# SciSharp/Gym.NET

Measured on AMD Instinct MI355X. Metric: env-steps/sec, higher is better.
Workload: dtype f32

## Files before the change

### gym.net_amd/build.py

```python
import os
import shutil
import subprocess

HERE = os.path.dirname(os.path.abspath(__file__))
CSRC = os.path.join(HERE, "csrc")
OUT = os.path.join(HERE, "lib", "libgymnet_amd.so")
SOURCES = ["env_cartpole.hip", "env_cartpole64.hip", "env_acrobot.hip", "env_pendulum.hip", "env_mountaincar.hip",
           "env_mountaincar_continuous.hip", "kernels.hip", "capi.hip", "launch_policy.hip", "resident.hip", "step_graph.hip",
           "group.hip", "render.hip", "pixel_stack.hip", "episode_memory.hip", "actor.hip", "actor_box.hip", "actor_box_policy.hip", "actor_box_logd.hip",
           "actor_softmax.hip", "actor_logp.hip", "actor_value.hip", "action_repeat.hip", "advantage.hip", "rollout_fused.hip"]
DEPS = SOURCES + ["kernels.hpp", "step_kernels.hpp", "lanes.hpp", "envs.hpp", "cartpole64.hpp", "philox.hpp", "handle.hpp", "launch_policy.hpp", "rollout_plan.hpp", "cartpole_raster.hpp", "actor_net.hpp", "actor_compose_logp.hpp", "actor_box_compose.hpp", "exp_neg.hpp", "log_pos.hpp", "advantage.hpp",
                  os.path.join("..", "..", "include", "gymnet_amd.h")]
FLAGS = ["--offload-arch=gfx950", "-O3", "-std=c++17", "-ffp-contract=off", "-fno-slp-vectorize", "-mllvm", "-amdgpu-kernarg-preload-count=14",
         "-fPIC", "-shared"]
LIBS = ["-ldl"]


def hipcc():
    exe = shutil.which("hipcc") or "/opt/rocm/bin/hipcc"
    if not os.path.exists(exe):
        raise RuntimeError("hipcc not found: cannot build the HIP extension")
    return exe


def up_to_date():
    if not os.path.exists(OUT):
        return False
    t = os.path.getmtime(OUT)
    return all(os.path.getmtime(os.path.join(CSRC, d)) <= t for d in DEPS)


def build(force=False, verbose=False):
    if not force and up_to_date():
        return OUT
    os.makedirs(os.path.dirname(OUT), exist_ok=True)
    import concurrent.futures
    import tempfile
    compile_flags = [f for f in FLAGS if f != "-shared"]
    with tempfile.TemporaryDirectory(prefix="gymnet_build_") as tmp:
        def compile_one(src):
            obj = os.path.join(tmp, os.path.splitext(src)[0] + ".o")
            cmd = [hipcc()] + compile_flags + ["-c", os.path.join(CSRC, src), "-o", obj]
            r = subprocess.run(cmd, capture_output=True, text=True)
            if r.returncode != 0:
                raise RuntimeError("hipcc failed:\n" + " ".join(cmd) + "\n" + r.stdout + r.stderr)
            return obj
        with concurrent.futures.ThreadPoolExecutor(max_workers=len(SOURCES)) as pool:
            objs = list(pool.map(compile_one, SOURCES))
        cmd = [hipcc(), "--offload-arch=gfx950", "-fPIC", "-shared"] + objs + LIBS + ["-o", OUT + ".tmp"]
        r = subprocess.run(cmd, capture_output=True, text=True)
        if r.returncode != 0:
            raise RuntimeError("hipcc (link) failed:\n" + " ".join(cmd) + "\n" + r.stdout + r.stderr)
    os.replace(OUT + ".tmp", OUT)
    if verbose:
        print("built", OUT)
    return OUT


if __name__ == "__main__":
    build(force=True, verbose=True)
```

### gym.net_amd/csrc/envs.hpp

```cpp
#pragma once
#include <hip/hip_runtime.h>
#include <stdint.h>

#include "philox.hpp"

namespace gymnet {


typedef float f2 __attribute__((ext_vector_type(2)));
namespace vm {
__device__ __forceinline__ float splat(float, float v) { return v; }
__device__ __forceinline__ f2 splat(f2, float v) { return f2{v, v}; }
__device__ __forceinline__ float fma(float a, float b, float c) { return fmaf(a, b, c); }
__device__ __forceinline__ f2 fma(f2 a, f2 b, f2 c) { return __builtin_elementwise_fma(a, b, c); }
template <class T> __device__ __forceinline__ T fmak(float k, T b, T c) { return fma(splat(b, k), b, c); }
template <class T> __device__ __forceinline__ T fmac(T a, T b, float k) { return fma(a, b, splat(a, k)); }
}

__device__ __forceinline__ void sincos_quadrant(float s, float c, float n, float &s_out, float &c_out) {
    const uint32_t q = (uint32_t)(int)n;
    const uint32_t q30 = q << 30, q31 = q << 31;
    const bool odd = (int32_t)q31 < 0;
    const float ss = odd ? c : s, cc = odd ? s : c;
    s_out = __uint_as_float(__builtin_amdgcn_bitop3_b32(__float_as_uint(ss), q30, 0x80000000u, 0x78));
    c_out = __uint_as_float(__builtin_amdgcn_bitop3_b32(__float_as_uint(cc), q30 ^ q31, 0x80000000u, 0x78));
}

template <class T>
__device__ __forceinline__ void sincos_bounded(T x, T &s_out, T &c_out) {
    T n;
    const T xs = x * vm::splat(x, 0.636619772367581343f);
    if constexpr (sizeof(T) == sizeof(float)) n = rintf(xs);
    else n = T{rintf(xs.x), rintf(xs.y)};
    T r = vm::fmak(-1.5703125f, n, x);
    r = vm::fmak(-4.837512969970703125e-4f, n, r);
    r = vm::fmak(-7.54978995489188216e-8f, n, r);
    const T z = r * r;
    T ps = vm::fmac(vm::splat(z, -1.9515295891e-4f), z, 8.3321608736e-3f);
    ps = vm::fmac(ps, z, -1.6666654611e-1f);
    const T s = vm::fma(r * z, ps, r);
    T pc = vm::fmac(vm::splat(z, 2.443315711809948e-5f), z, -1.388731625493765e-3f);
    pc = vm::fmac(pc, z, 4.166664568298827e-2f);
    const T c = vm::fma(z * z, pc, vm::fmac(vm::splat(z, -0.5f), z, 1.0f));
    if constexpr (sizeof(T) == sizeof(float)) {
        sincos_quadrant(s, c, n, s_out, c_out);
    } else {
        float s0, c0, s1, c1;
        sincos_quadrant(s.x, c.x, n.x, s0, c0);
        sincos_quadrant(s.y, c.y, n.y, s1, c1);
        s_out = T{s0, s1};
        c_out = T{c0, c1};
    }
}

template <class T>
__device__ __forceinline__ void sincos_small(T x, T &s_out, T &c_out) {
    T n;
    const T xs = x * vm::splat(x, 0.636619772367581343f);
    if constexpr (sizeof(T) == sizeof(float)) n = rintf(xs);
    else n = T{rintf(xs.x), rintf(xs.y)};
    T r = vm::fmak(-0x1.921fap+0f, n, x);
    r = vm::fmak(-0x1.54442ep-20f, n, r);
    const T z = r * r;
    T ps = vm::fmac(vm::splat(z, -1.9515295891e-4f), z, 8.3321608736e-3f);
    ps = vm::fmac(ps, z, -1.6666654611e-1f);
    const T s = vm::fma(r * z, ps, r);
    T pc = vm::fmac(vm::splat(z, 2.443315711809948e-5f), z, -1.388731625493765e-3f);
    pc = vm::fmac(pc, z, 4.166664568298827e-2f);
    pc = vm::fmac(pc, z, -0.5f);
    const T c = vm::fmac(pc, z, 1.0f);
    if constexpr (sizeof(T) == sizeof(float)) {
        sincos_quadrant(s, c, n, s_out, c_out);
    } else {
        float s0, c0, s1, c1;
        sincos_quadrant(s.x, c.x, n.x, s0, c0);
        sincos_quadrant(s.y, c.y, n.y, s1, c1);
        s_out = T{s0, s1};
        c_out = T{c0, c1};
    }
}

constexpr float kSmallAngle = 0.785f;
__device__ __forceinline__ void sincos_tiny(float x, float &s_out, float &c_out) {
    const float z = x * x;
    float ps = fmaf(-1.9515295891e-4f, z, 8.3321608736e-3f);
    ps = fmaf(ps, z, -1.6666654611e-1f);
// ... 38 lines not shown
    static constexpr const char *NAME = "CartPole";
    static constexpr int32_t ACTION_N = 2;

    static constexpr float gravity = 9.8f;
    static constexpr float masspole = 0.1f;
    static constexpr float total_mass = 0.1f + 1.0f;
    static constexpr float length = 0.5f;
    static constexpr float polemass_length = 0.1f * 0.5f;
    static constexpr float force_mag = 10.0f;
    static constexpr float tau = 0.02f;
    static constexpr float theta_threshold = 0.20943951606750488f;
    static constexpr float x_threshold = 2.4f;

    __device__ __forceinline__ static float div_tm(float x) { return DivByTotalMass<>::apply(x); }

    static constexpr bool HAS_SMALL_ANGLE_PATH = true;
    static constexpr int ANGLE_ROW = 2;
    static constexpr float SMALL_ANGLE_BOUND = kSmallAngle;

    template <bool SMALL_ANGLE = false, bool AUTORESET = false>
    __device__ __forceinline__ static void step(float (&s)[S], Action a, float &reward, bool &done) {
        const float x = s[0], x_dot = s[1], theta = s[2], theta_dot = s[3];
        const float s_in[S] = {x, x_dot, theta, theta_dot};
        const float force = (a == 1) ? force_mag : -force_mag;
        float sintheta, costheta;
        if constexpr (SMALL_ANGLE) sincos_tiny(theta, sintheta, costheta);
        else sincos_f32(theta, sintheta, costheta);
        const float temp = div_tm(force + polemass_length * theta_dot * theta_dot * sintheta);
        const float thetaacc = (gravity * sintheta - costheta * temp)
                               / (length * (4.0f / 3.0f - div_tm(masspole * costheta * costheta)));
        const float xacc = temp - div_tm(polemass_length * thetaacc * costheta);
        const float nx = x + tau * x_dot;
        const float nx_dot = x_dot + tau * xacc;
        const float ntheta = theta + tau * theta_dot;
        const float ntheta_dot = theta_dot + tau * thetaacc;
        s[0] = nx; s[1] = nx_dot; s[2] = ntheta; s[3] = ntheta_dot;
        bool term[DONE_TERMS];
        done_terms_of_inputs(s_in, term);
        done = term[0] || term[1];
        reward = 1.0f;
    }

    struct Pre {
        float x_dot, theta_dot;
        float nx, ntheta;
        float costheta;
        float centrifugal;
        float gsin;
        float divisor;
    };
    template <bool SMALL_ANGLE = false>
    __device__ __forceinline__ static void step_pre(const float (&s)[S], Pre &p) {
        const float x = s[0], x_dot = s[1], theta = s[2], theta_dot = s[3];
        float sintheta, costheta;
        if constexpr (SMALL_ANGLE) sincos_tiny(theta, sintheta, costheta);
        else sincos_f32(theta, sintheta, costheta);
        p.centrifugal = polemass_length * theta_dot * theta_dot * sintheta;
        p.gsin = gravity * sintheta;
        p.divisor = length * (4.0f / 3.0f - div_tm(masspole * costheta * costheta));
        p.costheta = costheta;
        p.nx = x + tau * x_dot;
        p.ntheta = theta + tau * theta_dot;
        p.x_dot = x_dot;
        p.theta_dot = theta_dot;
    }
    __device__ __forceinline__ static void step_post(const Pre &p, Action a, float (&s)[S], float &reward) { step_post(p, a == 1, s, reward); }
    __device__ __forceinline__ static void step_post(const Pre &p, bool right, float (&s)[S], float &reward) {
        const float force = right ? force_mag : -force_mag;
        const float temp = div_tm(force + p.centrifugal);
        const float thetaacc = (p.gsin - p.costheta * temp) / p.divisor;
        const float xacc = temp - div_tm(polemass_length * thetaacc * p.costheta);
        s[0] = p.nx; s[1] = p.x_dot + tau * xacc; s[2] = p.ntheta; s[3] = p.theta_dot + tau * thetaacc;
        reward = 1.0f;
    }

    static constexpr int DONE_TERMS = 2;
    __device__ __forceinline__ static void done_terms_of_inputs(const float (&s)[S], bool (&term)[DONE_TERMS]) {
        const double vx = __builtin_fma((double)tau, (double)s[1], (double)s[0]);
        const double vtheta = __builtin_fma((double)tau, (double)s[3], (double)s[2]);
        term[0] = __builtin_fabs(vx) > (double)x_threshold;
        term[1] = __builtin_fabs(vtheta) > (double)theta_threshold;
    }

    __device__ __forceinline__ static void reset(float (&s)[S], const PhiloxWords &r) {
#pragma unroll
        for (int k = 0; k < 4; ++k) s[k] = -0.05f + 0.1f * u01_24(r.w[k]);
    }

    __device__ __forceinline__ static void observe(const float (&s)[S], float (&o)[O]) {
#pragma unroll
        for (int k = 0; k < 4; ++k) o[k] = s[k];
    }
    __device__ __forceinline__ static void observe_fresh(const float (&s)[S], float (&o)[O]) { observe(s, o); }
    __device__ __forceinline__ static void step_observe(float (&s)[S], Action a, float &reward, bool &done, float (&o)[O]) {
        step(s, a, reward, done);
        observe(s, o);
    }
};

struct Pendulum {
    static constexpr int S = 2;
    static constexpr int O = 3;
    static constexpr bool OBS_ALIASES_STATE = false;
    static constexpr int OBS_ROW_OF_STATE[S] = {-1, 2};
    static constexpr bool HAS_SBD = false;
    static constexpr bool BOX_ACTION = true;
    static constexpr bool PACKED2 = false;
    static constexpr bool PIPE_LANES = false, PIPE_PAIRS = false;
    static constexpr bool HAS_SMALL_ANGLE_PATH = false;
    using Action = float;
    using Real = float;
    static constexpr bool RESET_TAKES_KEY = false;
    static constexpr const char *NAME = "Pendulum";
    static constexpr float ACTION_LOW = -2.0f, ACTION_HIGH = 2.0f;
    static constexpr float PI = 3.14159265358979323846f;

    __device__ __forceinline__ static float fmod_2pi(float a) {
        constexpr float m = 2.0f * PI, inv_m = 1.0f / m;
        const float ax = fabsf(a);
        if (__builtin_expect(!(ax < 4194304.0f * m), 0)) return fmodf(a, m);
        float q = truncf(ax * inv_m);
        float r = fmaf(-q, m, ax);
        q = r < 0.0f ? q - 1.0f : (r >= m ? q + 1.0f : q);
        r = fmaf(-q, m, ax);
        return copysignf(r, a);
    }

    __device__ __forceinline__ static float floored_mod_2pi(float a) {
        float r = fmod_2pi(a);
        if (r < 0.0f) r += 2.0f * PI;
        return r;
    }

    __device__ __forceinline__ static void step(float (&s)[S], Action a, float &reward, bool &done) {
        const float max_speed = 8.0f, max_torque = 2.0f, dt = 0.05f;
        const float th = s[0], thdot = s[1];
        const float u = a < -max_torque ? -max_torque : (a > max_torque ? max_torque : a);
        const float nrm = floored_mod_2pi(th + PI) - PI;
        const float costs = nrm * nrm + 0.1f * (thdot * thdot) + 0.001f * (u * u);
        float newthdot = thdot + (15.0f * sin_f32(th) + 3.0f * u) * dt;
        newthdot = newthdot < -max_speed ? -max_speed : (newthdot > max_speed ? max_speed : newthdot);
        const float newth = th + newthdot * dt;
        s[0] = newth; s[1] = newthdot;
        reward = -costs;
        done = false;
    }

    __device__ __forceinline__ static void reset(float (&s)[S], const PhiloxWords &r) {
        s[0] = -PI + (2.0f * PI) * u01_24(r.w[0]);
        s[1] = -1.0f + 2.0f * u01_24(r.w[1]);
    }

    __device__ __forceinline__ static void observe(const float (&s)[S], float (&o)[O]) {
        float sn, cs;
        sincos_f32(s[0], sn, cs);
        o[0] = cs; o[1] = sn; o[2] = s[1];
    }
    __device__ __forceinline__ static void observe_fresh(const float (&s)[S], float (&o)[O]) { observe(s, o); }
    __device__ __forceinline__ static void step_observe(float (&s)[S], Action a, float &reward, bool &done, float (&o)[O]) {
        step(s, a, reward, done);
        observe(s, o);
    }
};

struct MountainCar {
    static constexpr int S = 2;
// ... 231 lines not shown
```

### gym.net_amd/csrc/step_kernels.hpp

```cpp
#pragma once
#include "kernels.hpp"

#include <cstdio>
#include <type_traits>

#include "lanes.hpp"
#include "philox.hpp"

namespace gymnet {

__device__ __forceinline__ float abs_real(float x) { return fabsf(x); }
__device__ __forceinline__ double abs_real(double x) { return __builtin_fabs(x); }

template <class Env, bool UNIFORM_KEY = false>
__device__ __forceinline__ void draw_reset(typename Env::Real (&s)[Env::S], uint64_t key, uint64_t lane, uint64_t tick) {
    if constexpr (Env::RESET_TAKES_KEY) Env::reset(s, key, lane, tick);
    else Env::reset(s, lane_words<UNIFORM_KEY>(key, lane, tick));
}

template <class Env>
__device__ __forceinline__ constexpr bool state_row_own(int k) {
    if constexpr (Env::OBS_ALIASES_STATE) return true; else return Env::OBS_ROW_OF_STATE[k] < 0;
}
template <class Env>
// ... 2 lines not shown
    if constexpr (Env::OBS_ALIASES_STATE) return state + k * state_stride;
    else return Env::OBS_ROW_OF_STATE[k] < 0 ? state + k * state_stride : obs_in + Env::OBS_ROW_OF_STATE[k] * obs_stride;
}

__device__ __forceinline__ uint32_t wave_shard() {
    return (uint32_t)((((int64_t)blockIdx.x * blockDim.x + threadIdx.x) >> 6) & (kShards - 1));
}

template <int VEC, class Args>
__device__ __forceinline__ void count_after_done(const Args &a, const bool (&after)[VEC]) {
    uint32_t total = 0;
#pragma unroll
    for (int j = 0; j < VEC; ++j) total += (uint32_t)__popcll(__ballot(after[j]));
    if (total && lane_id() == (uint32_t)(__ffsll((unsigned long long)__ballot(1)) - 1))
        atomicAdd(&a.after_done[wave_shard() * kAfterStride], (unsigned long long)total);
}

template <class Env, bool AUTORESET, bool SMALL_ANGLE = false>
__device__ __forceinline__ void advance_sublane(typename Env::Real (&sj)[Env::S], typename Env::Action act, int32_t &sbd, float &rw,
                                                bool &dn, bool &after, bool in_range, typename Env::Real (&oj)[Env::O]) {
    if constexpr (Env::HAS_SMALL_ANGLE_PATH) Env::template step<SMALL_ANGLE, AUTORESET>(sj, act, rw, dn);
    else if constexpr (Env::OBS_ALIASES_STATE) Env::step(sj, act, rw, dn);
    else Env::step_observe(sj, act, rw, dn, oj);
    if constexpr (!AUTORESET && Env::HAS_SBD) {
        if (dn) {
            if (sbd == -1) { sbd = 0; }
            else { after = in_range; sbd += 1; rw = 0.0f; }
        }
    }
}

template <class Env, int VEC>
__device__ __forceinline__ bool wave_angles_small(const typename Env::Real (&s)[Env::S][VEC]) {
    if constexpr (!Env::HAS_SMALL_ANGLE_PATH) return false;
    else {
        bool small = true;
#pragma unroll
        for (int j = 0; j < VEC; ++j) small = small && (abs_real(s[Env::ANGLE_ROW][j]) <= Env::SMALL_ANGLE_BOUND);
        return __ballot(!small) == 0;
    }
}

template <class Env, int VEC, bool AUTORESET, bool GUARD, bool PACK = true>
__device__ __forceinline__ void advance_all(typename Env::Real (&s)[Env::S][VEC], typename Env::Action (&act)[VEC], int32_t (&sbd)[VEC],
                                            float (&rw)[VEC], bool (&dn)[VEC], bool (&after)[VEC], typename Env::Real (&o)[Env::O][VEC],
                                            int64_t i0, int64_t n) {
    constexpr int S = Env::S, O = Env::O;
    using Real = typename Env::Real;
#ifndef GYMNET_PROBE_NO_PACK
    constexpr bool kPack = true;
#else
    constexpr bool kPack = false;
#endif
    if constexpr (Env::PACKED2 && VEC == 2 && kPack && PACK) {
        Env::step_observe_x2(s, act, rw, dn, o);
    } else {
        auto all_sublanes = [&](auto small_tag) {
#pragma unroll
            for (int j = 0; j < VEC; ++j) {
                Real sj[S], oj[O];
#pragma unroll
                for (int k = 0; k < S; ++k) sj[k] = s[k][j];
                advance_sublane<Env, AUTORESET, decltype(small_tag)::value>(sj, act[j], sbd[j], rw[j], dn[j], after[j], !GUARD || i0 + j < n, oj);
#pragma unroll
                for (int k = 0; k < S; ++k) s[k][j] = sj[k];
                if constexpr (!Env::OBS_ALIASES_STATE) {
#pragma unroll
                    for (int k = 0; k < O; ++k) o[k][j] = oj[k];
                }
            }
        };
        if constexpr (Env::HAS_SMALL_ANGLE_PATH) {
            if (wave_angles_small<Env, VEC>(s)) all_sublanes(std::true_type{});
            else all_sublanes(std::false_type{});
        } else {
            all_sublanes(std::false_type{});
        }
    }
}

template <class Env, class = void> struct has_done_of_inputs : std::false_type {};
template <class Env> struct has_done_of_inputs<Env, std::void_t<decltype(&Env::done_terms_of_inputs)>> : std::true_type {};

template <class Env, class = void> struct has_split_step : std::false_type {};
template <class Env> struct has_split_step<Env, std::void_t<typename Env::Pre>> : std::true_type {};

template <class Env, int VEC>
__device__ __forceinline__ void pre_all_late_done(const typename Env::Real (&s)[Env::S][VEC], typename Env::Pre (&pre)[VEC], bool (&dn)[VEC],
                                                  uint64_t (&dmask)[VEC]) {
    constexpr int S = Env::S;
    using Real = typename Env::Real;
    static_assert(Env::HAS_SMALL_ANGLE_PATH && Env::OBS_ALIASES_STATE && has_done_of_inputs<Env>::value && has_split_step<Env>::value, "see above");
    auto all_sublanes = [&](auto small_tag) {
#pragma unroll
        for (int j = 0; j < VEC; ++j) {
            Real sj[S];
#pragma unroll
            for (int k = 0; k < S; ++k) sj[k] = s[k][j];
            Env::template step_pre<decltype(small_tag)::value>(sj, pre[j]);
        }
    };
    if (wave_angles_small<Env, VEC>(s)) all_sublanes(std::true_type{});
    else all_sublanes(std::false_type{});
#pragma unroll
    for (int j = 0; j < VEC; ++j) {
        Real wj[S];
#pragma unroll
        for (int k = 0; k < S; ++k) wj[k] = s[k][j];
        bool term[Env::DONE_TERMS];
        Env::done_terms_of_inputs(wj, term);
        bool any = false;
        uint64_t m = 0;
#pragma unroll
        for (int q = 0; q < Env::DONE_TERMS; ++q) { any = any || term[q]; m |= __builtin_amdgcn_ballot_w64(term[q]); }
        dn[j] = any;
        dmask[j] = m;
    }
}

template <class Env, int VEC>
__device__ __forceinline__ void post_all(const typename Env::Pre (&pre)[VEC], const typename Env::Action (&act)[VEC], const uint64_t (&dmask)[VEC],
                                         typename Env::Real (&s)[Env::S][VEC], float (&rw)[VEC]) {
    constexpr int S = Env::S;
    static_assert(std::is_same<typename Env::Action, int32_t>::value, "a discrete action");
    int32_t one = 1;
#pragma unroll
    for (int jj = 0; jj < VEC; ++jj) asm volatile("" : "+s"(one) : "v"(pre[jj].divisor), "s"(dmask[jj]));
#pragma unroll
    for (int j = 0; j < VEC; ++j) {
        typename Env::Real sj[S];
        Env::step_post(pre[j], act[j] == one, sj, rw[j]);
#pragma unroll
        for (int k = 0; k < S; ++k) s[k][j] = sj[k];
    }
}

template <class Env, int VEC, bool LANE_SEEDS>
__device__ __forceinline__ void reset_pending(uint32_t pending, typename Env::Real (&s)[Env::S][VEC], typename Env::Real (&o)[Env::O][VEC],
                                              const StepArgsT<typename Env::Real> &a, int64_t i0, int64_t n, uint64_t tick) {
    constexpr int S = Env::S, O = Env::O;
    using Real = typename Env::Real;
    while (pending) {
        const int j = __ffs(pending) - 1;
        pending &= pending - 1;
        Real sj[S];
        bool drawn = false;
        if constexpr (LANE_SEEDS) {
            if (a.lane_seed) {
                draw_reset<Env, false>(sj, i0 + j < n ? a.lane_seed[i0 + j] : a.seed, a.lane_offset + (uint64_t)(i0 + j), tick);
                drawn = true;
            }
        }
        if (!drawn) draw_reset<Env, true>(sj, a.seed, a.lane_offset + (uint64_t)(i0 + j), tick);
        Real oj[O];
        if constexpr (!Env::OBS_ALIASES_STATE) Env::observe_fresh(sj, oj);
#pragma unroll
        for (int jj = 0; jj < VEC; ++jj) {
            if (jj == j) {
#pragma unroll
                for (int k = 0; k < S; ++k) s[k][jj] = sj[k];
                if constexpr (!Env::OBS_ALIASES_STATE) {
#pragma unroll
                    for (int k = 0; k < O; ++k) o[k][jj] = oj[k];
                }
            }
        }
    }
}

template <class Env>
constexpr bool has_split_reset() { return Env::RESET_TAKES_KEY && Env::OBS_ALIASES_STATE; }

__device__ __forceinline__ PhiloxWords neighbour_words(const PhiloxWords &w) {
    PhiloxWords o;
#pragma unroll
    for (int k = 0; k < 4; ++k) o.w[k] = (uint32_t)__builtin_amdgcn_mov_dpp((int)w.w[k], 0xB1, 0xF, 0xF, true);
    return o;
}

#ifdef GYMNET_PROBE_RESET_MASKED
constexpr bool kResetFullExec = false;
#else
constexpr bool kResetFullExec = true;
#endif

template <class Env>
struct ResetScratch {
    uint32_t slot[64];
    typename Env::Real draw[64][Env::S];
};

__device__ __forceinline__ void wave_lds_fence() {
    __builtin_amdgcn_fence(__ATOMIC_RELEASE, "wavefront");
    __builtin_amdgcn_wave_barrier();
    __builtin_amdgcn_fence(__ATOMIC_ACQUIRE, "wavefront");
}

template <class Env, int VEC, bool LANE_SEEDS>
__device__ __forceinline__ void reset_pending_wave(uint32_t pending, typename Env::Real (&s)[Env::S][VEC], const StepArgsT<typename Env::Real> &a,
                                                   int64_t i0, int64_t n, uint64_t tick, ResetScratch<Env> *sc) {
// ... 28 lines not shown
        wave_lds_fence();
        if constexpr (SPLIT) {
            const uint32_t r = lane >> 1, call = lane & 1u;
            const bool draws = r < A && r < total - base;
            PhiloxWords w{};
            if (kResetFullExec || draws) {
                const uint32_t sl = sc->slot[draws ? r : 0u];
                const int64_t gl = wave_i0 + (int64_t)sl;
                uint64_t key = a.seed;
                if constexpr (LANE_SEEDS) {
                    if (a.lane_seed && gl < n) key = a.lane_seed[gl];
                }
                w = lane_words(Env::reset_call_key(key, call), a.lane_offset + (uint64_t)gl, tick);
            }
            const PhiloxWords other = neighbour_words(w);
            if ((kResetFullExec || draws) && call == 0) {
                Real sj[S];
                Env::reset_from_words(sj, w, other);
#pragma unroll
                for (int k = 0; k < S; ++k) sc->draw[r][k] = sj[k];
            }
        } else if (kResetFullExec || lane < total - base) {
            const uint32_t sl = sc->slot[lane < total - base ? lane : 0u];
            const int64_t gl = wave_i0 + (int64_t)sl;
            Real sj[S];
            bool drawn = false;
            if constexpr (LANE_SEEDS) {
                if (a.lane_seed) {
                    draw_reset<Env, false>(sj, gl < n ? a.lane_seed[gl] : a.seed, a.lane_offset + (uint64_t)gl, tick);
                    drawn = true;
                }
            }
            if (!drawn) draw_reset<Env, true>(sj, a.seed, a.lane_offset + (uint64_t)gl, tick);
#pragma unroll
            for (int k = 0; k < S; ++k) sc->draw[lane][k] = sj[k];
        }
        wave_lds_fence();
        Real got[VEC][S];
#pragma unroll
        for (int j = 0; j < VEC; ++j) {
            const uint32_t r = rank[j] - base;
#pragma unroll
            for (int k = 0; k < S; ++k) got[j][k] = sc->draw[r < A ? r : 0u][k];
        }
#pragma unroll
        for (int j = 0; j < VEC; ++j) {
            const bool mine = ((pending >> j) & 1u) && rank[j] - base < A;
#pragma unroll
            for (int k = 0; k < S; ++k) s[k][j] = mine ? got[j][k] : s[k][j];
        }
        wave_lds_fence();
    }
}

template <int VEC>
struct FinishedRanks {
    uint32_t rank[VEC];
    uint32_t total;
    bool single;
};

template <class Env, int VEC, bool LANE_SEEDS>
__device__ __forceinline__ void reset_finished_draw(const bool (&fin)[VEC], const uint64_t (&fmask)[VEC], const StepArgsT<typename Env::Real> &a,
                                                    int64_t wave_i0, int64_t n, uint64_t tick, ResetScratch<Env> *sc, FinishedRanks<VEC> &fr) {
    constexpr int S = Env::S;
    using Real = typename Env::Real;
    static_assert(Env::OBS_ALIASES_STATE && !has_split_reset<Env>(), "one-call resets that hand back the state only");
    const uint32_t lane = lane_id();
    uint32_t total = 0;
#pragma unroll
    for (int j = 0; j < VEC; ++j) {
        const uint64_t m = fmask[j];
        fr.rank[j] = total + __builtin_amdgcn_mbcnt_hi((uint32_t)(m >> 32), __builtin_amdgcn_mbcnt_lo((uint32_t)m, 0u));
        total += (uint32_t)__popcll(m);
    }
    fr.total = total;
    fr.single = !__builtin_expect(total == 0 || total > 64u || __ballot(1) != ~0ull, 0);
    if (!fr.single) return;
#pragma unroll
    for (int j = 0; j < VEC; ++j)
        if (fin[j]) sc->slot[fr.rank[j]] = lane * VEC + (uint32_t)j;
    wave_lds_fence();
    {
        const uint32_t sl = sc->slot[lane < total ? lane : 0u];
        const int64_t gl = wave_i0 + (int64_t)sl;
        Real sj[S];
        bool drawn = false;
        if constexpr (LANE_SEEDS) {
            if (a.lane_seed) {
                draw_reset<Env, false>(sj, gl < n ? a.lane_seed[gl] : a.seed, a.lane_offset + (uint64_t)gl, tick);
                drawn = true;
            }
        }
        if (!drawn) draw_reset<Env, true>(sj, a.seed, a.lane_offset + (uint64_t)gl, tick);
#pragma unroll
        for (int k = 0; k < S; ++k) sc->draw[lane][k] = sj[k];
    }
    wave_lds_fence();
}

template <class Env, int VEC>
__device__ __forceinline__ void reset_finished_take(const bool (&fin)[VEC], const FinishedRanks<VEC> &fr, typename Env::Real (&s)[Env::S][VEC],
                                                    ResetScratch<Env> *sc) {
    constexpr int S = Env::S;
    using Real = typename Env::Real;
    Real got[VEC][S];
#pragma unroll
    for (int j = 0; j < VEC; ++j) {
#pragma unroll
        for (int k = 0; k < S; ++k) got[j][k] = sc->draw[fr.rank[j] & 63u][k];
    }
#pragma unroll
    for (int j = 0; j < VEC; ++j) {
#pragma unroll
        for (int k = 0; k < S; ++k) s[k][j] = fin[j] ? got[j][k] : s[k][j];
    }
    wave_lds_fence();
}

template <class Env, int VEC, bool LANE_SEEDS>
__device__ __forceinline__ void reset_finished_rest(const bool (&fin)[VEC], const FinishedRanks<VEC> &fr, typename Env::Real (&s)[Env::S][VEC],
                                                    const StepArgsT<typename Env::Real> &a, int64_t i0, int64_t n, uint64_t tick, ResetScratch<Env> *sc) {
    if (fr.total == 0) return;
    uint32_t pending = 0;
#pragma unroll
    for (int j = 0; j < VEC; ++j) pending |= fin[j] ? (1u << j) : 0u;
    reset_pending_wave<Env, VEC, LANE_SEEDS>(pending, s, a, i0, n, tick, sc);
}

template <int VEC>
__device__ __forceinline__ uint32_t rank_finished(const bool (&finished)[VEC], uint32_t (&off)[VEC]) {
    uint32_t total = 0;
#pragma unroll
    for (int j = 0; j < VEC; ++j) {
        const uint64_t m = __ballot(finished[j]);
        off[j] = total + __builtin_amdgcn_mbcnt_hi((uint32_t)(m >> 32), __builtin_amdgcn_mbcnt_lo((uint32_t)m, 0u));
        total += (uint32_t)__popcll(m);
    }
    return total;
}

template <class Env, int VEC>
__device__ __forceinline__ void append_done_records(const StepArgsT<typename Env::Real> &a, const bool (&finished)[VEC], int64_t i0,
                                                    const typename Env::Real (&s)[Env::S][VEC], const typename Env::Real (&o)[Env::O][VEC],
                                                    const float (&fin_ret)[VEC], const int32_t (&fin_len)[VEC], bool stats) {
    constexpr int S = Env::S, O = Env::O;
    const uint32_t lane = lane_id();
    uint32_t off[VEC];
    const uint32_t total = rank_finished<VEC>(finished, off);
    if (total) {
        const int leader = __ffsll((unsigned long long)__ballot(1)) - 1;
        const uint32_t shard = wave_shard();
        uint32_t base = 0;
        if ((int)lane == leader)
            base = atomicAdd(&a.done_count2[a.cparity * (kShards * kCountStride) + shard * kCountStride], total);
        base = __shfl(base, leader);
        const int64_t seg0 = (int64_t)shard * a.done_cap;
#pragma unroll
        for (int j = 0; j < VEC; ++j) {
            if (!finished[j]) continue;
            const int64_t pos = seg0 + base + off[j];
            a.done_list[pos] = (int32_t)(i0 + j);
            if (stats) { a.rec_ret[pos] = fin_ret[j]; a.rec_len[pos] = fin_len[j]; }
            if (a.rec_obs) {
#pragma unroll
                for (int k = 0; k < O; ++k)
                    a.rec_obs[((int64_t)shard * O + k) * a.done_cap + base + off[j]] = Env::OBS_ALIASES_STATE ? s[k < S ? k : 0][j] : o[k][j];
// ... 102 lines not shown
                ep_len[j] += 1;
                if (a.max_episode_steps > 0 && ep_len[j] >= a.max_episode_steps) db |= 2;
            }
        }
        const bool fin = db != 0;
        finished[j] = fin && (!GUARD || i0 + j < n);
        done[j] = db;
        reward[j] = rw;

        if constexpr (EXTRAS) {
            if (fin && a.final_obs && (!GUARD || i0 + j < n)) {
#pragma unroll
                for (int k = 0; k < O; ++k) a.final_obs[k * n + i0 + j] = Env::OBS_ALIASES_STATE ? s[k < S ? k : 0][j] : o[k][j];
            }
            if (stats && fin && (!GUARD || i0 + j < n)) {
                fin_ret[j] = ep_ret[j];
                fin_len[j] = ep_len[j];
                if (a.fin_ret) { a.fin_ret[i0 + j] = ep_ret[j]; a.fin_len[i0 + j] = ep_len[j]; }
                if constexpr (AUTORESET) { ep_ret[j] = 0.0f; ep_len[j] = 0; }
            }
        }

        if constexpr (AUTORESET) pending |= fin ? (1u << j) : 0u;
    }

    if constexpr (!AUTORESET && Env::HAS_SBD) count_after_done<VEC>(a, after);

    store_f32<VEC, NT_O, GUARD>(a.reward, i0, n, reward);
    store_u8<VEC, NT_O, GUARD>(a.done, i0, n, done);

    if constexpr (EXTRAS) {
        if (a.done_list) append_done_records<Env, VEC>(a, finished, i0, s, o, fin_ret, fin_len, stats);
    }

    if constexpr (AUTORESET && RESETF == 1) reset_pending_wave<Env, VEC, EXTRAS>(pending, s, a, i0, n, tick, sc);
    else if constexpr (AUTORESET) reset_pending<Env, VEC, EXTRAS>(pending, s, o, a, i0, n, tick);

#pragma unroll
    for (int k = 0; k < S; ++k)
        if (state_row_own<Env>(k)) store_row<Real, VEC, NT_SS, GUARD>(a.state_out + k * a.state_stride, i0, n, s[k]);
    if constexpr (!Env::OBS_ALIASES_STATE) {
#pragma unroll
        for (int k = 0; k < O; ++k) store_row<Real, VEC, NT_SS, GUARD>(a.obs + k * a.obs_stride, i0, n, o[k]);
    }
    if constexpr (!AUTORESET && Env::HAS_SBD) store_i32<VEC, NT_SS, GUARD>(a.sbd, i0, n, sbd);

    if constexpr (EXTRAS) {
        if (stats) { store_f32<VEC, NT_SS, GUARD>(a.ep_ret, i0, n, ep_ret); store_i32<VEC, NT_SS, GUARD>(a.ep_len, i0, n, ep_len); }
    }
}

template <class Env, int VEC, bool AUTORESET, bool EXTRAS, int NT, bool GUARD, int RESETF = 0>
__device__ __forceinline__ void step_body(const StepArgsT<typename Env::Real> &a, const int64_t i0, const uint64_t tick, ResetScratch<Env> *sc = nullptr) {
    LaneInputs<Env, VEC> in;
    load_inputs<Env, VEC, AUTORESET, NT, GUARD>(a, i0, in);
    advance_and_store<Env, VEC, AUTORESET, EXTRAS, NT, GUARD, RESETF>(a, i0, tick, in, sc);
}

template <class Env, bool AUTORESET, bool EXTRAS>
constexpr bool has_full_workgroup_body() {
    return AUTORESET && !EXTRAS && Env::HAS_SMALL_ANGLE_PATH && Env::OBS_ALIASES_STATE && !has_split_reset<Env>() && has_done_of_inputs<Env>::value &&
           has_split_step<Env>::value;
}

template <class T>
__device__ __forceinline__ T *wg_row(T *row, const WgLanes &wg) { return wave_uniform(row + wg.first); }

#ifdef GYMNET_PROBE_RESET_BEHIND_ACTION
constexpr bool kResetDrawAhead = false;
#else
constexpr bool kResetDrawAhead = true;
#endif

template <class Env, int VEC, int NT, int RESETF>
__device__ __forceinline__ void step_body_wg(const StepArgsT<typename Env::Real> &a, const WgLanes wg, const uint64_t tick, ResetScratch<Env> *sc) {
    constexpr int S = Env::S;
    using Real = typename Env::Real;
    constexpr bool NT_SL = (NT & 1) != 0, NT_SS = (NT & 2) != 0, NT_A = (NT & 4) != 0, NT_O = (NT & 8) != 0;
    static_assert(!Env::BOX_ACTION && Env::OBS_ALIASES_STATE, "a discrete-action env whose observation is its state");
    const int64_t i0 = wg.first + (int64_t)wg.local;

    Real s[S][VEC];
    typename Env::Action act[VEC];
#pragma unroll
    for (int k = 0; k < S; ++k) load_row_wg<Real, VEC, NT_SL>(wg_row(static_cast<const Real *>(a.state) + k * a.state_stride, wg), wg.local, s[k]);
    load_row_wg<int32_t, VEC, NT_A>(wg_row(static_cast<const int32_t *>(a.action), wg), wg.local, act);

    typename Env::Pre pre[VEC];
    bool finished[VEC];
    uint64_t fmask[VEC];
    pre_all_late_done<Env, VEC>(s, pre, finished, fmask);

    float reward[VEC];
    auto store_reward_done = [&] {
        const uint32_t local = reissued(wg.local);
        store_row_wg<float, VEC, NT_O>(wg_row(a.reward, wg), local, reward);
        uint32_t w = 0;
#pragma unroll
        for (int j = 0; j < VEC; ++j) w |= finished[j] ? (1u << (8 * j)) : 0u;
        store_done_word_wg<VEC, NT_O>(wg_row(a.done, wg), local, w);
    };

    if constexpr (RESETF == 1 && kResetDrawAhead) {
        FinishedRanks<VEC> fr;
        reset_finished_draw<Env, VEC, false>(finished, fmask, a, wg.first + (int64_t)__builtin_amdgcn_readfirstlane(wg.local), a.n, tick, sc, fr);
        if (fr.single) {
            post_all<Env, VEC>(pre, act, fmask, s, reward);
            reset_finished_take<Env, VEC>(finished, fr, s, sc);
        } else {
            post_all<Env, VEC>(pre, act, fmask, s, reward);
            reset_finished_rest<Env, VEC, false>(finished, fr, s, a, wg.first + (int64_t)reissued(wg.local), a.n, tick, sc);
        }
        store_reward_done();
    } else {
        post_all<Env, VEC>(pre, act, fmask, s, reward);
        store_reward_done();
        if constexpr (RESETF == 1) {
            FinishedRanks<VEC> fr;
            reset_finished_draw<Env, VEC, false>(finished, fmask, a, wg.first + (int64_t)__builtin_amdgcn_readfirstlane(wg.local), a.n, tick, sc, fr);
            if (fr.single) reset_finished_take<Env, VEC>(finished, fr, s, sc);
            else reset_finished_rest<Env, VEC, false>(finished, fr, s, a, i0, a.n, tick, sc);
        } else {
            uint32_t pending = 0;
#pragma unroll
            for (int j = 0; j < VEC; ++j) pending |= finished[j] ? (1u << j) : 0u;
            Real o_unused[Env::O][VEC];
            reset_pending<Env, VEC, false>(pending, s, o_unused, a, i0, a.n, tick);
        }
    }

    const uint32_t local = reissued(wg.local);
#pragma unroll
    for (int k = 0; k < S; ++k) store_row_wg<Real, VEC, NT_SS>(wg_row(a.state_out + k * a.state_stride, wg), local, s[k]);
}

template <class Env>
struct LaneOutputs { typename Env::Real s[Env::S], o[Env::O]; float reward; uint8_t done; int32_t sbd; };

template <class Env, bool AUTORESET>
__device__ __forceinline__ void compute_lane(const StepArgsT<typename Env::Real> &a, int64_t i, uint64_t tick, LaneInputs<Env, 1> &in,
                                             LaneOutputs<Env> &out) {
    constexpr int S = Env::S, O = Env::O;
    typename Env::Real o[O][1];
    float rw[1];
    bool dn[1], after[1] = {false};
    advance_all<Env, 1, AUTORESET, false>(in.s, in.act, in.sbd, rw, dn, after, o, i, a.n);
    if constexpr (!AUTORESET && Env::HAS_SBD) count_after_done<1>(a, after);
    if constexpr (AUTORESET) reset_pending<Env, 1, false>(dn[0] ? 1u : 0u, in.s, o, a, i, a.n, tick);
#pragma unroll
    for (int k = 0; k < S; ++k) out.s[k] = in.s[k][0];
#pragma unroll
    for (int k = 0; k < O; ++k) out.o[k] = o[k][0];
    out.reward = rw[0]; out.done = dn[0] ? 1 : 0; out.sbd = in.sbd[0];
}

template <class Env, bool AUTORESET, int NT>
__device__ __forceinline__ void store_lane(const StepArgsT<typename Env::Real> &a, int64_t i, const LaneOutputs<Env> &out) {
    constexpr bool NT_SS = (NT & 2) != 0, NT_O = (NT & 8) != 0;
    auto st = [](auto *p, auto v, bool nt) { if (nt) __builtin_nontemporal_store(v, p); else *p = v; };
    st(a.reward + i, out.reward, NT_O);
    if constexpr (NT_O) __builtin_nontemporal_store(out.done, a.done + i); else a.done[i] = out.done;
#pragma unroll
    for (int k = 0; k < Env::S; ++k)
        if (state_row_own<Env>(k)) st(a.state_out + k * a.state_stride + i, out.s[k], NT_SS);
    if constexpr (!Env::OBS_ALIASES_STATE) {
#pragma unroll
        for (int k = 0; k < Env::O; ++k) st(a.obs + k * a.obs_stride + i, out.o[k], NT_SS);
    }
// ... 202 lines not shown
    const uint64_t tick = a.tick2[a.parity];
    if (blockIdx.x == 0 && threadIdx.x == 0) a.tick2[a.parity ^ 1] = tick + 1;
    const int lane = threadIdx.x & 63;
    const bool storer = (threadIdx.x >> 6) == kLdsComputeWaves;
    const int cl = threadIdx.x;
    const int64_t t0 = (int64_t)blockIdx.x * TPB;
    const int nt = (int)(tiles - t0 < TPB ? tiles - t0 : TPB);

    auto tile_barrier = [] { asm volatile("s_waitcnt lgkmcnt(0)\n\ts_barrier" ::: "memory"); };

    LaneInputs<Env, 1> in[TPB + 1];
    if (!storer) load_inputs<Env, 1, AUTORESET, NT, false>(a, t0 * kLdsTile + cl, in[0]);
#pragma unroll
    for (int s = 0; s <= TPB; ++s) {
        if (!storer) {
            if (s < TPB) {
                const int64_t i = (t0 + (s < nt ? s : nt - 1)) * kLdsTile + cl;
                const int64_t ip = (t0 + (s + 1 < nt ? s + 1 : nt - 1)) * kLdsTile + cl;
                load_inputs<Env, 1, AUTORESET, NT, false>(a, ip, in[s + 1]);
#pragma unroll
                for (int c = 0; c < S; ++c) asm volatile("" : "+v"(in[s].s[c][0]));
                asm volatile("" : "+v"(in[s].act[0]));
                LaneOutputs<Env> out;
                compute_lane<Env, AUTORESET>(a, i, tick, in[s], out);
#pragma unroll
                for (int c = 0; c < S; ++c) asm volatile("" : "+v"(in[s + 1].s[c][0]), "+v"(out.s[S - 1]));
                asm volatile("" : "+v"(in[s + 1].act[0]), "+v"(out.reward));
                if (s < nt) {
                    int r = 0;
#pragma unroll
                    for (int k = 0; k < S; ++k)
                        if (state_row_own<Env>(k)) out_buf[s & 1][r++][cl] = out.s[k];
                    if constexpr (!Env::OBS_ALIASES_STATE) {
#pragma unroll
                        for (int k = 0; k < O; ++k) out_buf[s & 1][r++][cl] = out.o[k];
                    }
                    out_buf[s & 1][r][cl] = out.reward;
                    done_buf[s & 1][cl] = out.done;
                }
            }
        } else if (s >= 1 && s - 1 < nt) {
            const int b = (s - 1) & 1;
            const int64_t base = (t0 + s - 1) * kLdsTile;
            auto drain = [&](float *row, int r, bool nt_store) {
#pragma unroll
                for (int j = 0; j < kLdsTile / 256; ++j) {
                    const f32x4 v = *reinterpret_cast<const f32x4 *>(&out_buf[b][r][j * 256 + lane * 4]);
                    f32x4 *dst = reinterpret_cast<f32x4 *>(row + base + j * 256 + lane * 4);
                    if (nt_store) __builtin_nontemporal_store(v, dst); else *dst = v;
                }
                static_assert(kLdsTile % 256 == 0, "the storing wave moves 256 floats per instruction");
            };
            int r = 0;
#pragma unroll
            for (int k = 0; k < S; ++k)
                if (state_row_own<Env>(k)) drain(a.state_out + k * a.state_stride, r++, NT_SS);
            if constexpr (!Env::OBS_ALIASES_STATE) {
#pragma unroll
                for (int k = 0; k < O; ++k) drain(a.obs + k * a.obs_stride, r++, NT_SS);
            }
            drain(a.reward, r, NT_O);
            if (lane < kLdsTile / 16) {
                const i32x4 v = *reinterpret_cast<const i32x4 *>(&done_buf[b][lane * 16]);
                i32x4 *dst = reinterpret_cast<i32x4 *>(a.done + base + lane * 16);
                if constexpr (NT_O) __builtin_nontemporal_store(v, dst); else *dst = v;
            }
        }
        tile_barrier();
    }
}

template <class Env, int VEC, bool AUTORESET, bool EXTRAS, int NT, int RESETF = 0>
__global__ __launch_bounds__(256) void step_kernel(typename Env::Real *state, const void *action, int64_t n, int64_t state_stride, uint64_t *tick2,
                                                   float *reward, int32_t block, int32_t parity, const StepArgsT<typename Env::Real> rest) {
    const StepArgsT<typename Env::Real> a = hot_step_args(state, action, n, state_stride, tick2, reward, parity, rest);
    const WgLanes wg{(int64_t)blockIdx.x * block * VEC, (uint32_t)threadIdx.x * (uint32_t)VEC};
    const int64_t i0 = wg.first + (int64_t)wg.local;
    ResetScratch<Env> *sc = nullptr;
    if constexpr (RESETF == 1) {
        __shared__ ResetScratch<Env> scratch[256 / 64];
        sc = &scratch[threadIdx.x >> 6];
    }
    const uint64_t tick = a.tick2[a.parity];
    if (blockIdx.x == 0 && threadIdx.x == 0) {
        a.tick2[a.parity ^ 1] = tick + 1;
    }
    if constexpr (EXTRAS) {
        if (blockIdx.x == 0 && a.done_count2)
            for (int sh = threadIdx.x; sh < kShards; sh += block) a.done_count2[(a.cparity ^ 1) * (kShards * kCountStride) + sh * kCountStride] = 0u;
    }
    if (((int64_t)blockIdx.x + 1) * block * VEC <= a.n) {
        if constexpr (has_full_workgroup_body<Env, AUTORESET, EXTRAS>()) step_body_wg<Env, VEC, NT, RESETF>(a, wg, tick, sc);
        else step_body<Env, VEC, AUTORESET, EXTRAS, NT, false, RESETF>(a, i0, tick, sc);
    } else {
        if (i0 >= a.n) return;
        step_body<Env, VEC, AUTORESET, EXTRAS, NT, true, RESETF>(a, i0, tick, sc);
    }
}

template <class Env>
__device__ __forceinline__ typename Env::Action sampled_action(uint32_t word_a) {
    if constexpr (Env::BOX_ACTION) return Env::ACTION_LOW + (Env::ACTION_HIGH - Env::ACTION_LOW) * u01_24(word_a);
    else return (int32_t)__umulhi(word_a, (uint32_t)Env::ACTION_N);
}

template <int VEC>
__device__ __forceinline__ void thread_action_words(uint64_t seed, uint64_t gl0, uint64_t tick, bool want_aux, bool one_group,
                                                    uint32_t (&wa)[VEC], uint32_t (&wb)[VEC]) {
    static_assert(VEC == 1 || VEC == 2 || VEC == 4, "a thread's lanes must fit one group of four");
    if (one_group) {
        const PhiloxWords r = action_group_words<true>(seed, gl0 >> 2, tick);
        PhiloxWords c{};
        if (want_aux) c = aux_group_words<true>(seed, gl0 >> 2, tick);
        const uint32_t base = (uint32_t)gl0 & 3u;
        if constexpr (VEC == 4) {
#pragma unroll
            for (int j = 0; j < 4; ++j) { wa[j] = r.w[j]; wb[j] = c.w[j]; }
        } else if constexpr (VEC == 2) {
#pragma unroll
            for (int j = 0; j < 2; ++j) { wa[j] = base ? r.w[2 + j] : r.w[j]; wb[j] = base ? c.w[2 + j] : c.w[j]; }
        } else {
            wa[0] = word_of(r, base); wb[0] = word_of(c, base);
        }
    } else {
#pragma unroll
        for (int j = 0; j < VEC; ++j) { wa[j] = 0u; wb[j] = 0u; }
#pragma unroll 1
        for (int j = 0; j < VEC; ++j) {
            const uint32_t a = action_word<true>(seed, gl0 + (uint64_t)j, tick);
            const uint32_t b = want_aux ? aux_word<true>(seed, gl0 + (uint64_t)j, tick) : 0u;
#pragma unroll
            for (int k = 0; k < VEC; ++k) { wa[k] = k == j ? a : wa[k]; wb[k] = k == j ? b : wb[k]; }
        }
    }
}

constexpr uint32_t kStageRecords = 256;
struct EpisodeStage { int32_t t[kStageRecords], lane[kStageRecords]; float ret[kStageRecords]; int32_t len[kStageRecords]; };

struct NoHook { static constexpr bool CHOOSES = false; };

struct NoRepeat { static constexpr bool ON = false; };
struct HeldAction { static constexpr bool ON = true; int32_t R; };

template <class Env, int VEC, bool AUTORESET, bool GUARD, bool EXTRAS, bool SAMPLE, int RESETF = 0, int RECORDS = 0, class Hook = NoHook, class Rep = NoRepeat>
__device__ __forceinline__ void rollout_body(const StepArgsT<typename Env::Real> &a, const RolloutArgsT<typename Env::Real> &ro,
                                             const int64_t i0, const uint64_t tick0, ResetScratch<Env> *sc = nullptr, EpisodeStage *stage = nullptr,
                                             Hook hook = Hook{}, Rep rep = Rep{}) {
    static_assert(!Rep::ON || (!Hook::CHOOSES && !(Env::PACKED2 && VEC == 2)), "frame skip: ring / sampled actions, unpacked sub-lanes");
    constexpr int S = Env::S, O = Env::O;
    using Act = typename Env::Action;
    using Real = typename Env::Real;
    const int64_t n = a.n;

    Real s[S][VEC];
#pragma unroll
    for (int k = 0; k < S; ++k) load_row<Real, VEC, true, GUARD>(state_row_src<Env>(a.state, a.state_stride, a.obs_in, a.obs_stride, k), i0, n, s[k]);
    int32_t sbd[VEC] = {};
    if constexpr (!AUTORESET && Env::HAS_SBD) load_i32<VEC, true, GUARD>(a.sbd, i0, n, sbd);

    auto load_action = [&](int64_t slice, Act (&dst)[VEC]) {
        const char *base = static_cast<const char *>(a.action) + (size_t)(slice * ro.action_stride) * 4;
        if constexpr (Env::BOX_ACTION) load_f32<VEC, true, GUARD>(reinterpret_cast<const float *>(base), i0, n, dst);
        else load_i32<VEC, true, GUARD>(reinterpret_cast<const int32_t *>(base), i0, n, dst);
    };

// ... 603 lines not shown
```

Baseline: 166.0 billion.

## Filter CartPole done checks in f32 with exact f64 fallback; streamline step prologue

```diff
diff --git a/gym.net_amd/build.py b/gym.net_amd/build.py
--- a/gym.net_amd/build.py
+++ b/gym.net_amd/build.py
@@ -9,7 +9,7 @@
            "env_mountaincar_continuous.hip", "kernels.hip", "capi.hip", "launch_policy.hip", "resident.hip", "step_graph.hip",
            "group.hip", "render.hip", "pixel_stack.hip", "episode_memory.hip", "actor.hip", "actor_box.hip", "actor_box_policy.hip", "actor_box_logd.hip",
            "actor_softmax.hip", "actor_logp.hip", "actor_value.hip", "action_repeat.hip", "advantage.hip", "rollout_fused.hip"]
-DEPS = SOURCES + ["kernels.hpp", "step_kernels.hpp", "lanes.hpp", "envs.hpp", "cartpole64.hpp", "philox.hpp", "handle.hpp", "launch_policy.hpp", "rollout_plan.hpp", "cartpole_raster.hpp", "actor_net.hpp", "actor_compose_logp.hpp", "actor_box_compose.hpp", "exp_neg.hpp", "log_pos.hpp", "advantage.hpp",
+DEPS = SOURCES + ["kernels.hpp", "step_kernels.hpp", "lanes.hpp", "envs.hpp", "cartpole_done_filter.hpp", "cartpole64.hpp", "philox.hpp", "handle.hpp", "launch_policy.hpp", "rollout_plan.hpp", "cartpole_raster.hpp", "actor_net.hpp", "actor_compose_logp.hpp", "actor_box_compose.hpp", "exp_neg.hpp", "log_pos.hpp", "advantage.hpp",
                   os.path.join("..", "..", "include", "gymnet_amd.h")]
 FLAGS = ["--offload-arch=gfx950", "-O3", "-std=c++17", "-ffp-contract=off", "-fno-slp-vectorize", "-mllvm", "-amdgpu-kernarg-preload-count=14",
          "-fPIC", "-shared"]
diff --git a/gym.net_amd/csrc/cartpole_done_filter.hpp b/gym.net_amd/csrc/cartpole_done_filter.hpp
--- /dev/null
+++ b/gym.net_amd/csrc/cartpole_done_filter.hpp
@@ -0,0 +1,30 @@
+#pragma once
+
+#if defined(__HIPCC__) || defined(__CUDACC__)
+#define GYMNET_FILTER_HD __host__ __device__ __forceinline__
+#else
+#define GYMNET_FILTER_HD inline
+#endif
+
+namespace gymnet {
+
+struct CartPoleDoneBand {
+    static constexpr float x_threshold = 2.4f, x_ulp = 0x1p-22f;
+    static constexpr float theta_threshold = 0.20943951606750488f, theta_ulp = 0x1p-26f;
+    static constexpr float x_lo = x_threshold - 4.0f * x_ulp, x_hi = x_threshold + 4.0f * x_ulp;
+    static constexpr float theta_lo = theta_threshold - 4.0f * theta_ulp, theta_hi = theta_threshold + 4.0f * theta_ulp;
+};
+
+GYMNET_FILTER_HD void cartpole_done_compares(float p0, float w, float lo, float hi, bool &inside, bool &below, bool &above) {
+    const float a0 = __builtin_fabsf(p0), aw = __builtin_fabsf(w);
+    inside = a0 < lo;
+    below = aw < lo;
+    above = aw > hi;
+}
+GYMNET_FILTER_HD bool cartpole_done_term_f32(float p0, float w, float lo, float hi, bool &done) {
+    bool inside, below;
+    cartpole_done_compares(p0, w, lo, hi, inside, below, done);
+    return inside && (below || done);
+}
+
+}
diff --git a/gym.net_amd/csrc/envs.hpp b/gym.net_amd/csrc/envs.hpp
--- a/gym.net_amd/csrc/envs.hpp
+++ b/gym.net_amd/csrc/envs.hpp
@@ -2,6 +2,7 @@
 #include <hip/hip_runtime.h>
 #include <stdint.h>
 
+#include "cartpole_done_filter.hpp"
 #include "philox.hpp"
 
 namespace gymnet {
@@ -206,6 +207,21 @@
         term[1] = __builtin_fabs(vtheta) > (double)theta_threshold;
     }
 
+    __device__ __forceinline__ static void done_terms_filter(const float (&s)[S], const Pre &p, bool (&inside)[DONE_TERMS], bool (&below)[DONE_TERMS],
+                                                             bool (&above)[DONE_TERMS]) {
+        using B = CartPoleDoneBand;
+        static_assert(B::x_threshold == x_threshold && B::theta_threshold == theta_threshold, "one pair of thresholds");
+        cartpole_done_compares(s[0], p.nx, B::x_lo, B::x_hi, inside[0], below[0], above[0]);
+        cartpole_done_compares(s[2], p.ntheta, B::theta_lo, B::theta_hi, inside[1], below[1], above[1]);
+    }
+
+#ifdef GYMNET_PROBE_STEP_CHAIN
+    __device__ __forceinline__ static void done_terms_rounded(const Pre &p, bool (&term)[DONE_TERMS]) {
+        term[0] = fabsf(p.nx) > x_threshold;
+        term[1] = fabsf(p.ntheta) > theta_threshold;
+    }
+#endif
+
     __device__ __forceinline__ static void reset(float (&s)[S], const PhiloxWords &r) {
 #pragma unroll
         for (int k = 0; k < 4; ++k) s[k] = -0.05f + 0.1f * u01_24(r.w[k]);
diff --git a/gym.net_amd/csrc/step_kernels.hpp b/gym.net_amd/csrc/step_kernels.hpp
--- a/gym.net_amd/csrc/step_kernels.hpp
+++ b/gym.net_amd/csrc/step_kernels.hpp
@@ -108,8 +108,19 @@
 template <class Env, class = void> struct has_done_of_inputs : std::false_type {};
 template <class Env> struct has_done_of_inputs<Env, std::void_t<decltype(&Env::done_terms_of_inputs)>> : std::true_type {};
 
+#ifdef GYMNET_PROBE_STEP_CHAIN
+constexpr int kProbeStepChain = GYMNET_PROBE_STEP_CHAIN;
+constexpr bool kStepChainShipped = false;
+#else
+constexpr int kProbeStepChain = 0;
+constexpr bool kStepChainShipped = true;
+#endif
+
 template <class Env, class = void> struct has_split_step : std::false_type {};
 template <class Env> struct has_split_step<Env, std::void_t<typename Env::Pre>> : std::true_type {};
+
+template <class Env, class = void> struct has_done_filter : std::false_type {};
+template <class Env> struct has_done_filter<Env, std::void_t<decltype(&Env::done_terms_filter)>> : std::true_type {};
 
 template <class Env, int VEC>
 __device__ __forceinline__ void pre_all_late_done(const typename Env::Real (&s)[Env::S][VEC], typename Env::Pre (&pre)[VEC], bool (&dn)[VEC],
@@ -128,20 +139,52 @@
     };
     if (wave_angles_small<Env, VEC>(s)) all_sublanes(std::true_type{});
     else all_sublanes(std::false_type{});
-#pragma unroll
-    for (int j = 0; j < VEC; ++j) {
-        Real wj[S];
-#pragma unroll
-        for (int k = 0; k < S; ++k) wj[k] = s[k][j];
-        bool term[Env::DONE_TERMS];
-        Env::done_terms_of_inputs(wj, term);
-        bool any = false;
-        uint64_t m = 0;
-#pragma unroll
-        for (int q = 0; q < Env::DONE_TERMS; ++q) { any = any || term[q]; m |= __builtin_amdgcn_ballot_w64(term[q]); }
-        dn[j] = any;
-        dmask[j] = m;
-    }
+    auto exact_flags = [&] {
+#pragma unroll
+        for (int j = 0; j < VEC; ++j) {
+            Real wj[S];
+#pragma unroll
+            for (int k = 0; k < S; ++k) wj[k] = s[k][j];
+            bool term[Env::DONE_TERMS];
+            if constexpr ((kProbeStepChain & 1) != 0) Env::done_terms_rounded(pre[j], term);
+            else Env::done_terms_of_inputs(wj, term);
+            bool any = false;
+            uint64_t m = 0;
+#pragma unroll
+            for (int q = 0; q < Env::DONE_TERMS; ++q) { any = any || term[q]; m |= __builtin_amdgcn_ballot_w64(term[q]); }
+            dn[j] = any;
+            dmask[j] = m;
+        }
+    };
+    if constexpr (has_done_filter<Env>::value && kStepChainShipped) {
+        uint64_t undecided = 0;
+        uint64_t above_mask[VEC];
+        bool any_above[VEC];
+#pragma unroll
+        for (int j = 0; j < VEC; ++j) {
+            Real wj[S];
+#pragma unroll
+            for (int k = 0; k < S; ++k) wj[k] = s[k][j];
+            bool inside[Env::DONE_TERMS], below[Env::DONE_TERMS], above[Env::DONE_TERMS];
+            Env::done_terms_filter(wj, pre[j], inside, below, above);
+            uint64_t m = 0;
+            bool any = false;
+#pragma unroll
+            for (int q = 0; q < Env::DONE_TERMS; ++q) {
+                const uint64_t hi = __builtin_amdgcn_ballot_w64(above[q]);
+                undecided |= ~(__builtin_amdgcn_ballot_w64(inside[q]) & (__builtin_amdgcn_ballot_w64(below[q]) | hi));
+                m |= hi;
+                any = any || above[q];
+            }
+            above_mask[j] = m;
+            any_above[j] = any;
+        }
+        if (__builtin_expect((undecided & __builtin_amdgcn_ballot_w64(true)) != 0, 0)) exact_flags();
+        else {
+#pragma unroll
+            for (int j = 0; j < VEC; ++j) { dmask[j] = above_mask[j]; dn[j] = any_above[j]; }
+        }
+    } else exact_flags();
 }
 
 template <class Env, int VEC>
@@ -336,7 +379,7 @@
         if (fin[j]) sc->slot[fr.rank[j]] = lane * VEC + (uint32_t)j;
     wave_lds_fence();
     {
-        const uint32_t sl = sc->slot[lane < total ? lane : 0u];
+        const uint32_t sl = (kProbeStepChain & 4) != 0 ? lane : sc->slot[lane < total ? lane : 0u];
         const int64_t gl = wave_i0 + (int64_t)sl;
         Real sj[S];
         bool drawn = false;
@@ -605,8 +648,17 @@
 
     Real s[S][VEC];
     typename Env::Action act[VEC];
-#pragma unroll
-    for (int k = 0; k < S; ++k) load_row_wg<Real, VEC, NT_SL>(wg_row(static_cast<const Real *>(a.state) + k * a.state_stride, wg), wg.local, s[k]);
+    if constexpr (kStepChainShipped) {
+        const Real *row = wg_row(static_cast<const Real *>(a.state), wg);
+#pragma unroll
+        for (int k = 0; k < S; ++k) {
+            load_row_wg<Real, VEC, NT_SL>(row, wg.local, s[k]);
+            row = wave_uniform(row + a.state_stride);
+        }
+    } else {
+#pragma unroll
+        for (int k = 0; k < S; ++k) load_row_wg<Real, VEC, NT_SL>(wg_row(static_cast<const Real *>(a.state) + k * a.state_stride, wg), wg.local, s[k]);
+    }
     load_row_wg<int32_t, VEC, NT_A>(wg_row(static_cast<const int32_t *>(a.action), wg), wg.local, act);
 
     typename Env::Pre pre[VEC];
@@ -975,6 +1027,36 @@
         sc = &scratch[threadIdx.x >> 6];
     }
     const uint64_t tick = a.tick2[a.parity];
+    if constexpr ((kProbeStepChain & 2) != 0 && has_full_workgroup_body<Env, AUTORESET, EXTRAS>() && VEC == 4 && RESETF == 1) {
+        StepArgsT<typename Env::Real> b = a;
+        b.state_stride = (int64_t)(uint32_t)state_stride;
+        const WgLanes wg32{(int64_t)((uint32_t)blockIdx.x * (uint32_t)block * (uint32_t)VEC), (uint32_t)threadIdx.x * (uint32_t)VEC};
+        step_body_wg<Env, VEC, NT, RESETF>(b, wg32, tick, sc);
+        if (blockIdx.x == 0 && threadIdx.x == 0) a.tick2[a.parity ^ 1] = tick + 1;
+        return;
+    }
+    if constexpr (kStepChainShipped && has_full_workgroup_body<Env, AUTORESET, EXTRAS>()) {
+        const uint32_t wg_lanes = (uint32_t)block * (uint32_t)VEC;
+        const uint64_t first = (uint64_t)(uint32_t)blockIdx.x * (uint64_t)wg_lanes;
+        const uint64_t room = (uint64_t)n - (first + wg_lanes);
+        const WgLanes wgu{(int64_t)first, (uint32_t)threadIdx.x * (uint32_t)VEC};
+        uint32_t room_hi = (uint32_t)(room >> 32);
+        asm volatile("" : "+s"(room_hi));
+        auto write_next_tick = [&] {
+            if (blockIdx.x == 0) {
+                asm volatile("");
+                if (threadIdx.x == 0) a.tick2[a.parity ^ 1] = tick + 1;
+            }
+        };
+        if (__builtin_expect((int32_t)room_hi < 0, 0)) {
+            if (wgu.first + (int64_t)wgu.local < a.n) step_body<Env, VEC, AUTORESET, EXTRAS, NT, true, RESETF>(a, wgu.first + (int64_t)wgu.local, tick, sc);
+            write_next_tick();
+            return;
+        }
+        step_body_wg<Env, VEC, NT, RESETF>(a, wgu, tick, sc);
+        write_next_tick();
+        return;
+    }
     if (blockIdx.x == 0 && threadIdx.x == 0) {
         a.tick2[a.parity ^ 1] = tick + 1;
     }
```

Result: faster. 168.7 billion (median of 6 runs) (+1.6%).
